# loryruta/gl-radix-sort

Hardware: AMD Instinct MI355X
Metric: Mkeys/s sorting 2^28 uint32 key+val; % HBM roofline; 1/2/4/8 GPU (higher is better)
Workload: dtype u32; 1 GPU; 2^28 uint32 key + uint32 val pairs, uniform-random full-range keys, vals=iota, in-place stable radix sort, 1x MI355X; pairs_per_gpu=268435456, key_distribution=uniform, parallelism=single, device=AMD Radeon Graphics (gfx950:sramecc+:xnack-), 256 CUs, 288.0 GiB, device 0

## Files before the change

### gl-radix-sort_amd/csrc/glu_hip.hip

```cpp
#include <hip/hip_runtime.h>

#include <algorithm>
#include <chrono>
#include <cmath>
#include <cstdarg>
#include <cstdio>
#include <cstdlib>
#include <cstring>
#include <mutex>
#include <string>
#include <strings.h>
#include <unordered_map>
#include <vector>

#include "glu_host.hpp"
#include "glu_sort_launch.hpp"
#include "glu_sort_object.hpp"
#include "radix_sort_kernels.hpp"
#include "radix_scatter_lines.hpp"
#include "radix_pair_passes.hpp"
#include "radix_seg_passes.hpp"
#include "radix_lds_plan.hpp"

using namespace glu_hip;
// ... 284 lines not shown
                else if (!(seen & 7u) && s->finish_backoff)
                    s->finish_wait = s->finish_backoff;
            }
        }
        if (s->finish_wait)
        {
            s->finish_wait--;
            finish_kpt = 0;
        }
    }
    if (finish_kpt)
    {
        s->finish_seq = s->finish_seq >= 0x0FFFFFFFu ? 1u : s->finish_seq + 1;
        s->cur_seq = s->finish_seq;
        for (uint32_t i = num_passes; i-- > 0;) passes[i + 2] = passes[i];
        finish_top_bit = !device_top && key_xf == KEY_XF_NONE && !s->no_bit_shortcut && s->finish_top ? std::min<uint32_t>(s->finish_top, end_bit) : end_bit;
        passes[0] = PassDesc{finish_top_bit - 16u, 8u, key_xf, 0};
        passes[1] = PassDesc{finish_top_bit - 8u, 8u, 0u, 0};
        num_passes += 2;
    }
    const bool finish_long_ok = finish_kpt && s->long_runs && s->long_image.ptr && finish_top_bit >= 16 &&
                                finish_top_bit - 16u <= (sizeof(KeyT) == 4 ? 16u : 48u);
    s->last_finish_long_ok = finish_long_ok;
    s->last_device_top = finish_kpt && device_top;
    s->last_finish_top = finish_kpt ? finish_top_bit : 0u;
    s->last_finish_attempted = finish_kpt != 0;
    const uint32_t finish_last = std::min<uint32_t>(finish_kpt + 2, kFinishGeometries);
    const uint32_t finish_expected = s->finish_last_geo >= finish_kpt && s->finish_last_geo <= finish_last ? s->finish_last_geo : finish_kpt;
    s->last_finish_capacity = finish_kpt ? finish_geometry_capacity(finish_last) : 0u;
    if (pairs_ok || finish_kpt)
    {
        const bool lines8 = lines_applicable<KeyT, 8>(s, kbuf[0], vbuf[0], kbuf[1], vbuf[1], count);
        const bool lines4 = lines_applicable<KeyT, 4>(s, kbuf[0], vbuf[0], kbuf[1], vbuf[1], count);
        for (uint32_t i = 0; i + 1 < num_passes;)
        {
            const bool wide = passes[i].bits > 4;
            if ((pairs_ok || (finish_kpt && i == 0)) && wide == (passes[i + 1].bits > 4) && (wide ? lines8 : lines4) &&
                ((passes[i].xform & 3u) == 0 || (finish_kpt && i == 0)))
            {
                passes[i].pair_role = 1;
                passes[i + 1].pair_role = 2;
                i += 2;
            }
            else
                i += 1;
        }
    }
    if (planned)
    {
        PassPlan* plan = (PassPlan*) s->plan.ptr;
        static_assert(offsetof(PassPlan, sample_done) + sizeof(plan->sample_done) <= sizeof(PassPlan) && offsetof(PassPlan, sample_done) + 64 > sizeof(PassPlan),
                      "sample_done is the last member of the zeroed tail of the plan");
        static_assert(offsetof(PassPlan, pair_fallback) % 64 == 0 && sizeof(PassPlan) % 64 == 0, "one aligned fill");
        HIP_TRY(hipMemsetAsync(plan->pair_fallback, 0, sizeof(PassPlan) - offsetof(PassPlan, pair_fallback), stream));
        if (finish_kpt && device_top)
        {
            hipLaunchKernelGGL((radix_sample_top_kernel<KeyT>), dim3(kSampleTopBlocks), dim3(256), 0, stream, (const KeyT*) kbuf[0], (uint32_t) count, end_bit,
                               std::min<uint32_t>(s->top_floor, end_bit), plan);
            HIP_TRY(hipGetLastError());
        }
    }
    if (planned)
        for (uint32_t i = 0; i < (uint32_t) kPlanMaxPasses; i++) s->last_pair_roles[i] = i < num_passes ? (uint32_t) passes[i].pair_role : 0u;
    const bool fork = planned && finish_kpt && s->fork_behind && !s->finish_last_refused && s->ensure_side();
    uint32_t pass = 0;
    for (; pass < num_passes; pass++)
    {
        const uint32_t shift = passes[pass].shift, bits = passes[pass].bits, xform = passes[pass].xform;
        if (planned)
        {
            PlanArgs pa;
            pa.plan = (PassPlan*) s->plan.ptr;
            pa.pass = pass;
            pa.may_skip = xform == 0;
            if (key_xf == KEY_XF_NONE && !s->no_bit_shortcut) pa.flags = pass == 0 ? kPlanCollectBits : (pa.may_skip ? kPlanShortcut : 0u);
            pa.pair_role = passes[pass].pair_role;
            if (pa.pair_role == 1)
            {
                pa.shift2 = passes[pass + 1].shift;
                pa.bits2 = passes[pass + 1].bits;
            }
            s->cur_kind = finish_kpt && pass < 2 ? 1 : 0;
            pa.behind_attempt = finish_kpt && pass >= 2;
            s->cur_behind = pa.behind_attempt;
            if (finish_kpt && pass == 0)
            {
                pa.finish_geo_first = finish_kpt;
                pa.finish_geo_last = finish_last;
                pa.finish_first_ordinary = 2;
                pa.finish_num_ordinary = num_passes - 2;
                pa.finish_seq = s->finish_seq;
                pa.finish_top_bit = finish_top_bit;
                pa.finish_key_bits = end_bit;
                pa.finish_long_ok = finish_long_ok;
                pa.fork_side = fork;
            }
            pa.unitsum_side = fork && pass == 1 && pa.pair_role == 2 && bits == 8;
            GLU_TRY(dispatch_pass<KeyT>(s, kbuf[0], vbuf[0], kbuf[1], vbuf[1], count, shift, bits, nullptr,
                                        fork && pa.behind_attempt ? s->side : stream, xform, pa));
            {
                if (finish_kpt && pass == 1)
                {
                    if (fork) HIP_TRY(hipEventRecord(s->ev_fork2, stream));
                    s->cur_kind = 2;
                    s->cur_behind = false;
                    s->mark(stream);
                    s->mark(stream);
                    const FinishMarks finish_marks{[](void* object, hipStream_t st) { ((glu_radix_sort_s*) object)->mark(st, true); }, s};
// ... 1162 lines not shown
```

### gl-radix-sort_amd/csrc/glu_sort_passes.hpp

```cpp
#pragma once
#include "glu_sort_object.hpp"
#include "radix_scatter_lines.hpp"
#include "radix_pair_passes.hpp"
#include "radix_lds_plan.hpp"

namespace glu_hip
{
namespace host
{
template<typename KeyT, int BITS, bool LARGE, bool XF, bool VALS>
glu_status launch_pass(glu_radix_sort_s* s, const KeyT* src_k, const uint32_t* src_v, KeyT* dst_k, uint32_t* dst_v,
                       size_t count, uint32_t shift, uint32_t bits, uint32_t* histogram_out, hipStream_t stream,
                       uint32_t xform = 0, PlanArgs pa = PlanArgs())
{
    using G = GeometryFor<KeyT, BITS, LARGE, VALS>;
    constexpr int RADIX = 1 << BITS;
    const uint32_t tiles = (uint32_t) ((count + G::TILE - 1) / G::TILE);
    uint64_t cap = (uint64_t) usable_cus(s) * G::BLOCKS_PER_CU;
    if (s->max_blocks) cap = std::min<uint64_t>(cap, s->max_blocks);
    const uint32_t nb = (uint32_t) std::max<uint64_t>(1, std::min<uint64_t>(tiles, cap));
    const uint32_t mask = (1u << bits) - 1;
    uint32_t* table = (uint32_t*) s->table.ptr;
    uint32_t* totals = table + (size_t) RADIX * nb;

// ... 106 lines not shown
            }
            else
            {
                auto count4_plain = radix_pair4_count_kernel<KeyT, G::TILE, false, false>;
                auto count4_collect = radix_pair4_count_kernel<KeyT, G::TILE, false, true>;
                hipLaunchKernelGGL((pa.flags & kPlanCollectBits) ? count4_collect : count4_plain,
                                   dim3(nb * kPairSub), dim3(256), 0, stream, src_k, sub_table, (uint32_t*) s->pair_t2.ptr, (uint32_t) count, shift, mask, pa.shift2,
                                   (1u << pa.bits2) - 1, tiles, xform, (const KeyT*) dst_k, pa.plan, pa.pass, pa.flags, share);
            }
            HIP_TRY(hipGetLastError());
        }
    }
    if (pa.pair_role == 2)
    {
        uint32_t* leader_table = table;
        table = (uint32_t*) s->pair_table.ptr;
        totals = table + (size_t) RADIX * nb;
        ranges = (const uint2*) s->pair_ranges.ptr;
        if constexpr (BITS == 8)
        {
            hipLaunchKernelGGL(radix_pair_unitsum_kernel, dim3(nb), dim3(1024), 0, pa.unitsum_side ? s->side : stream, (const uint32_t*) s->pair_t2.ptr,
                               (const uint32_t*) leader_table, (const uint32_t*) (leader_table + (size_t) RADIX * nb), table,
                               (uint2*) s->pair_ranges.ptr, (uint32_t) count, pa.plan, pa.pass, shift, mask, pa.flags);
            if (pa.unitsum_side)
            {
                HIP_TRY(hipEventRecord(s->ev_unit, s->side));
                HIP_TRY(hipStreamWaitEvent(stream, s->ev_unit, 0));
            }
        }
        else
            hipLaunchKernelGGL(radix_pair4_unitsum_kernel, dim3(nb), dim3(1024), 0, stream, (const uint32_t*) s->pair_t2.ptr,
                               (const uint32_t*) sub_table, (const uint32_t*) (leader_table + (size_t) RADIX * nb), table,
                               (uint2*) s->pair_ranges.ptr, (uint32_t) count, pa.plan, pa.pass, shift, mask, pa.flags);
        HIP_TRY(hipGetLastError());
    }
    if (pa.pair_role != 1)
    {
        auto count_plain = radix_count_kernel<KeyT, BITS, 1024, G::TILE, XF, false>;
        auto count_collect = radix_count_kernel<KeyT, BITS, 1024, G::TILE, XF, !XF>;
        hipLaunchKernelGGL((pa.flags & kPlanCollectBits) ? count_collect : count_plain, dim3(nb), dim3(1024), 0, stream, src_k, table,
                           (uint32_t) count, shift, mask, tiles, xform, (const KeyT*) dst_k, pa.plan, pa.pass, pa.pair_role == 2,
                           pa.flags, share);
        HIP_TRY(hipGetLastError());
    }
    s->mark(stream);
    if (BITS == 4 && pa.pair_role == 1)
    {
        hipLaunchKernelGGL((radix_row_scan_kernel<256>), dim3(RADIX), dim3(256), 0, stream, sub_table, totals, nb * kPairSub,
                           (uint32_t) count, pa.may_skip ? pa.plan : (PassPlan*) nullptr, pa.pass, 0u, pa.plan, table,
                           kPairSub);
    }
    else
    {
        hipLaunchKernelGGL((radix_row_scan_kernel<256>), dim3(RADIX), dim3(256), 0, stream, table, totals, nb, (uint32_t) count,
                           pa.may_skip ? pa.plan : (PassPlan*) nullptr, pa.pass,
                           pa.pair_role == 1 && BITS == 8
                               ? (s->pair_unit_div ? std::max<uint32_t>(1u, (uint32_t) (count / nb / s->pair_unit_div)) : 0xFFFFFFFFu)
                               : 0u,
                           pa.plan);
    }
    HIP_TRY(hipGetLastError());
    if (pa.finish_geo_first)
    {
        hipLaunchKernelGGL(radix_finish_lengths_kernel, dim3(kPairRadix), dim3(1024), 0, stream, (const uint32_t*) s->pair_t2.ptr, nb,
                           (uint32_t*) s->finish_lengths.ptr, (const PassPlan*) pa.plan, pa.pass, (const uint32_t*) s->pair_wide.ptr);
        HIP_TRY(hipGetLastError());
        const bool long_runs = pa.finish_long_ok && s->long_image.ptr;
        hipLaunchKernelGGL(radix_finish_plan_kernel, dim3(kFinishPlanBlocks), dim3(1024), 0, stream, (const uint32_t*) s->finish_lengths.ptr,
                           (uint32_t*) s->finish_starts.ptr, (uint32_t) count, pa.finish_geo_first, pa.finish_geo_last, pa.plan, pa.pass,
                           pa.finish_first_ordinary, pa.finish_num_ordinary, s->finish_hint, pa.finish_seq, pa.finish_top_bit,
                           pa.finish_key_bits, long_runs ? 1u : 0u, (uint32_t*) s->finish_crowded.ptr, (uint32_t*) s->finish_outcomes.ptr,
                           (uint32_t) (sizeof(KeyT) + (VALS ? sizeof(uint32_t) : 0)));
        HIP_TRY(hipGetLastError());
        if (long_runs)
        {
            hipLaunchKernelGGL(radix_finish_long_runs_kernel, dim3(1), dim3(1024), 0, stream, (const uint32_t*) s->finish_starts.ptr,
                               (const PassPlan*) pa.plan, usable_cus(s) * kLongRunsSharesPerWg, (uint32_t*) s->long_image.ptr, (uint32_t*) s->long_hdr.ptr);
            HIP_TRY(hipGetLastError());
        }
        if (pa.fork_side)
        {
            HIP_TRY(hipEventRecord(s->ev_fork, stream));
            HIP_TRY(hipStreamWaitEvent(s->side, s->ev_fork, 0));
        }
    }
    s->mark(stream, true);
    if (histogram_out)
    {
        HIP_TRY(hipMemcpyAsync(histogram_out, totals, ((size_t) 1 << bits) * sizeof(uint32_t), hipMemcpyDeviceToDevice,
                               stream));
        if (s->after_histogram_event) HIP_TRY(hipEventRecord(s->after_histogram_event, stream));
    }
    hipLaunchKernelGGL(scatter, dim3(nb), dim3(G::THREADS), sizeof(Smem), stream, src_k, src_v, dst_k, dst_v,
                       (const uint32_t*) table, (const uint32_t*) totals, (uint32_t) count, shift, mask, tiles,
                       (unsigned long long*) nullptr, xform, pa.plan, pa.pass, ranges, share, (const uint32_t*) nullptr, (const uint32_t*) nullptr, 0u, 0u, (const uint32_t*) nullptr);
    s->mark(stream, true);
    HIP_TRY(hipGetLastError());
    return GLU_OK;
}

template<typename KeyT, int BITS>
glu_status launch_pass_sized(glu_radix_sort_s* s, const KeyT* src_k, const uint32_t* src_v, KeyT* dst_k, uint32_t* dst_v,
                             size_t count, uint32_t shift, uint32_t bits, uint32_t* histogram_out, hipStream_t stream,
                             uint32_t xform = 0, PlanArgs pa = PlanArgs())
{
    const bool vals = src_v != nullptr;
    const size_t large_tile = vals ? GeometryFor<KeyT, BITS, true, true>::TILE : GeometryFor<KeyT, BITS, true, false>::TILE;
    const bool large = count >= large_tiles_from<KeyT, BITS>(s, vals, large_tile) && !s->force_small;
    {
        if (lines_applicable<KeyT, BITS>(s, src_k, src_v, dst_k, dst_v, count))
        {
#define GLU_LAUNCH_LINES(XF_, VALS_) \
    launch_pass_lines<KeyT, BITS, XF_, VALS_>(s, src_k, src_v, dst_k, dst_v, count, shift, bits, histogram_out, stream, XF_ ? xform : 0u, pa)
            if (vals) return xform ? GLU_LAUNCH_LINES(true, true) : GLU_LAUNCH_LINES(false, true);
            return xform ? GLU_LAUNCH_LINES(true, false) : GLU_LAUNCH_LINES(false, false);
#undef GLU_LAUNCH_LINES
        }
    }
#define GLU_LAUNCH(LARGE_, XF_, VALS_) \
// ... 22 lines not shown
```

### gl-radix-sort_amd/csrc/radix_lds_plan.hpp

```cpp
#pragma once

#include "radix_lds_finish.hpp"
#include "radix_pair_passes.hpp"

namespace glu_hip
{
constexpr uint32_t kSampleTopBlocks = 64;
template<typename KeyT>
__global__ __launch_bounds__(256) void radix_sample_top_kernel(const KeyT* __restrict__ keys, uint32_t n, uint32_t key_bits,
                                                               uint32_t floor_top, PassPlan* plan)
{
    typedef uint32_t u32x4_t __attribute__((ext_vector_type(4)));
    __shared__ uint32_t red[4][4];
    const uint32_t tid = threadIdx.x, lane = tid & 63, wave = tid >> 6;
    constexpr uint32_t W = sizeof(KeyT) / 4;
    const uint64_t nvec = (uint64_t) n * sizeof(KeyT) / 16;
    const uint32_t total = gridDim.x * 256u;
    const uint32_t samples = (uint32_t) (nvec < total ? nvec : total);
    const uint64_t stride = samples ? nvec / samples : 1;
    uint32_t o[2] = {0, 0}, no[2] = {0, 0};
    const uint32_t j = blockIdx.x * 256u + tid;
    if (j < samples)
    {
        const u32x4_t x = reinterpret_cast<const u32x4_t*>(keys)[(uint64_t) j * stride];
        if (W == 1)
        {
            o[0] = x.x | x.y | x.z | x.w;
            no[0] = ~x.x | ~x.y | ~x.z | ~x.w;
        }
        else
        {
            o[0] = x.x | x.z;
            no[0] = ~x.x | ~x.z;
            o[1] = x.y | x.w;
            no[1] = ~x.y | ~x.w;
        }
    }
    if (blockIdx.x == 0 && tid == 0 && n)
    {
        const KeyT f = keys[0], l = keys[n - 1];
        o[0] |= (uint32_t) f | (uint32_t) l;
        no[0] |= ~(uint32_t) f | ~(uint32_t) l;
        if (W == 2)
        {
            o[1] |= (uint32_t) ((uint64_t) f >> 32) | (uint32_t) ((uint64_t) l >> 32);
            no[1] |= ~(uint32_t) ((uint64_t) f >> 32) | ~(uint32_t) ((uint64_t) l >> 32);
        }
    }
#pragma unroll
    for (int s = 32; s > 0; s >>= 1)
    {
        o[0] |= __shfl_xor(o[0], s);
        o[1] |= __shfl_xor(o[1], s);
        no[0] |= __shfl_xor(no[0], s);
        no[1] |= __shfl_xor(no[1], s);
    }
    if (lane == 0) red[0][wave] = o[0], red[1][wave] = o[1], red[2][wave] = no[0], red[3][wave] = no[1];
    __syncthreads();
    if (tid == 0)
    {
        for (int w = 1; w < 4; w++) o[0] |= red[0][w], o[1] |= red[1][w], no[0] |= red[2][w], no[1] |= red[3][w];
        __hip_atomic_fetch_or(&plan->sample_or[0], o[0], __ATOMIC_RELAXED, __HIP_MEMORY_SCOPE_AGENT);
        __hip_atomic_fetch_or(&plan->sample_nor[0], no[0], __ATOMIC_RELAXED, __HIP_MEMORY_SCOPE_AGENT);
        if (W == 2)
        {
            __hip_atomic_fetch_or(&plan->sample_or[1], o[1], __ATOMIC_RELAXED, __HIP_MEMORY_SCOPE_AGENT);
            __hip_atomic_fetch_or(&plan->sample_nor[1], no[1], __ATOMIC_RELAXED, __HIP_MEMORY_SCOPE_AGENT);
        }
        const uint32_t done = __hip_atomic_fetch_add(&plan->sample_done, 1u, __ATOMIC_ACQ_REL, __HIP_MEMORY_SCOPE_AGENT);
        if (done + 1 == gridDim.x)
        {
            const uint32_t vo0 = __hip_atomic_load(&plan->sample_or[0], __ATOMIC_RELAXED, __HIP_MEMORY_SCOPE_AGENT);
            const uint32_t vn0 = __hip_atomic_load(&plan->sample_nor[0], __ATOMIC_RELAXED, __HIP_MEMORY_SCOPE_AGENT);
            const uint32_t vo1 = W == 2 ? __hip_atomic_load(&plan->sample_or[1], __ATOMIC_RELAXED, __HIP_MEMORY_SCOPE_AGENT) : 0u;
            const uint32_t vn1 = W == 2 ? __hip_atomic_load(&plan->sample_nor[1], __ATOMIC_RELAXED, __HIP_MEMORY_SCOPE_AGENT) : 0u;
            const uint64_t varying = (uint64_t) (vo0 & vn0) | ((uint64_t) (vo1 & vn1) << 32);
            uint32_t top = varying ? 64u - (uint32_t) __builtin_clzll(varying) : 0u;
            top = max(max(top, floor_top), 16u);
            top = min(top, key_bits);
            if (W == 2 && top > 32 && top < 48 && top != 40) top = top < 40 ? 40u : 48u;
            plan->top_bit = top;
            plan->shift_down[0] = plan->shift_down[1] = key_bits - top;
        }
    }
}

constexpr uint32_t kLongRunsMax = 8192;
constexpr uint32_t kLongRunsMinShare = 4096;
constexpr uint32_t kLongRunsSharesPerWg = 8;

struct LongRunsLayout
{
    uint32_t nwg, off_first, off_list, off_start, words;
    __host__ __device__ explicit LongRunsLayout(uint32_t nwg_) : nwg(nwg_)
    {
        off_first = 2u * (kLongRunsMax + nwg);
        off_list = off_first + nwg + 1u;
        off_start = off_list + kLongRunsMax + 1u;
        words = off_start + kLongRunsMax;
    }
};
__device__ __forceinline__ void finish_list_long_runs(const uint32_t* starts, uint32_t geo, uint32_t finish_longest, uint32_t nwg ,
                                                      uint32_t* __restrict__ image, uint32_t* __restrict__ hdr, uint32_t (&wsum)[2][16])
{
    const LongRunsLayout lay(nwg);
    const uint32_t tid = threadIdx.x, lane = tid & 63, wave = tid >> 6;
    const uint32_t cap = finish_geometry_capacity(geo);
    constexpr uint32_t PER = kFinishRuns / 1024;
    auto ld = [&](uint32_t i) { return starts[i]; };
    if (geo == 0 || finish_longest <= cap)
    {
        if (tid < 4) hdr[tid] = tid < 3 ? 0u : nwg;
        return;
    }
    for (uint32_t w = tid; w <= nwg; w += 1024) image[lay.off_first + w] = 0xFFFFFFFFu;
    uint32_t cnt = 0, len = 0;
    {
        uint32_t a = ld(tid * PER);
        for (uint32_t j = 0; j < PER; j++)
        {
            const uint32_t e = ld(tid * PER + j + 1);
            if (e - a > cap) cnt++, len += e - a;
            a = e;
        }
    }
    auto block_exclusive = [&](uint32_t v, int slot, uint32_t& total) -> uint32_t {
        uint32_t wtotal;
        uint32_t excl = wave_exclusive_sum(v, lane, wtotal);
// ... 26 lines not shown
    const uint32_t per_wg = (uint32_t) min<uint64_t>(kLongRunsSharesPerWg, max<uint64_t>(1ull, (uint64_t) total * 64ull / ((uint64_t) finish_longest * wgs)));
    nwg = wgs * per_wg;
    if (tid == 0) hdr[3] = nwg;
    const uint32_t share = max((total + nwg - 1) / nwg, kLongRunsMinShare);
    uint32_t subs = 0;
    {
        uint32_t a = ld(tid * PER), p = pos;
        for (uint32_t j = 0; j < PER; j++)
        {
            const uint32_t e = ld(tid * PER + j + 1), l = e - a;
            if (l > cap)
            {
                subs += (p + l - 1) / share - p / share + 1;
                p += l;
            }
            a = e;
        }
    }
    uint32_t nsb;
    uint32_t sb = block_exclusive(subs, 0, nsb);
    {
        uint32_t a = ld(tid * PER), p = pos, g = seg;
        for (uint32_t j = 0; j < PER; j++)
        {
            const uint32_t e = ld(tid * PER + j + 1), l = e - a;
            if (l > cap)
            {
                image[lay.off_list + g] = sb;
                image[lay.off_start + g] = a;
                for (uint32_t w = p / share; w <= (p + l - 1) / share; w++)
                {
                    const uint32_t b0 = max(p, w * share), b1 = min(p + l, (w + 1) * share);
                    image[2 * sb] = a + (b0 - p);
                    image[2 * sb + 1] = a + (b1 - p);
                    if (b0 == w * share) image[lay.off_first + w] = sb;
                    sb++;
                }
                p += l;
                g++;
            }
            a = e;
        }
    }
    __syncthreads();
    if (tid == 0)
    {
        hdr[1] = nsb;
        image[lay.off_list + nseg] = nsb;
    }
    for (uint32_t w = tid; w <= nwg; w += 1024)
        if (image[lay.off_first + w] == 0xFFFFFFFFu) image[lay.off_first + w] = nsb;
}

static __global__ __launch_bounds__(1024) void radix_finish_lengths_kernel(const uint32_t* __restrict__ t2, uint32_t nb,
                                                                    uint32_t* __restrict__ lengths, const PassPlan* plan,
                                                                    uint32_t pass, const uint32_t* __restrict__ wide = nullptr)
{
    if (plan->off[pass] || plan->skip[pass] == kSkipWithoutCounting) return;
    __shared__ uint32_t part[8][kPairRadix];
    __shared__ uint32_t wide_list[1024], wide_n;
    const uint32_t tid = threadIdx.x, g = tid >> 7, q = tid & 127u, d = blockIdx.x;
    uint32_t lo = 0, hi = 0;
#pragma unroll 4
    for (uint32_t b = g; b < nb; b += 8)
    {
        const uint32_t w = t2[((size_t) d * nb + b) * kPairRowWords + q];
        lo += w & 0xFFFFu;
        hi += w >> 16;
    }
    part[g][2 * q] = lo;
    part[g][2 * q + 1] = hi;
    if (tid == 0) wide_n = 0;
    __syncthreads();
    if (wide && tid < nb)
    {
        const uint32_t* hdr = wide + (size_t) tid * kPairWideStride;
        const uint32_t nw = hdr[0] <= kPairWideRows ? hdr[0] : 0u;
        for (uint32_t k = 0; k < nw; k++)
            if (hdr[1 + k] == d) wide_list[atomicAdd(&wide_n, 1u)] = (tid << 8) | k;
    }
    __syncthreads();
    if (tid < kPairRadix)
    {
        uint32_t c = 0;
#pragma unroll
        for (int k = 0; k < 8; k++) c += part[k][tid];
        for (uint32_t i = 0; i < wide_n; i++)
        {
            const uint32_t bk = wide_list[i];
            c += wide[(size_t) (bk >> 8) * kPairWideStride + 16 + (bk & 255u) * kPairRadix + tid] << 16;
        }
        lengths[tid * kPairRadix + d] = c;
    }
}

static __global__ __launch_bounds__(1024) void radix_finish_plan_kernel(const uint32_t* __restrict__ lengths, uint32_t* starts,
                                                                 uint32_t n, uint32_t geo_first, uint32_t geo_last, PassPlan* plan,
                                                                 uint32_t pass,
                                                                 uint32_t first_ordinary, uint32_t num_ordinary,
                                                                 uint32_t* hint, uint32_t attempt, uint32_t top_bit,
                                                                 uint32_t key_bits, uint32_t long_ok, uint32_t* crowded_lists,
                                                                 uint32_t* outcomes = nullptr, uint32_t pair_bytes = 8)
{
    __shared__ uint32_t tmp[3][16];
    __shared__ uint32_t over_tmp[2][kFinishGeometries][16];
    const uint32_t tid = threadIdx.x, lane = tid & 63, wave = tid >> 6, b = blockIdx.x;
    const bool tables = !(plan->off[pass] || plan->skip[pass] == kSkipWithoutCounting);
    uint32_t before = 0, all = 0, longest = 0, mine = 0;
    uint32_t over_len[kFinishGeometries] = {}, over_cnt[kFinishGeometries] = {};
    if (tables)
    {
#pragma unroll
        for (uint32_t j = 0; j < kFinishPlanBlocks; j++)
        {
            const uint32_t v = lengths[j * 1024u + tid];
            all += v;
            before += j < b ? v : 0u;
            longest = max(longest, v);
            mine = j == b ? v : mine;
            if (long_ok && b == 0)
            {
#pragma unroll
                for (uint32_t g = 0; g < kFinishGeometries; g++)
                {
                    const bool over = v > finish_geometry_capacity(g + 1);
                    over_len[g] += over ? v : 0u;
                    over_cnt[g] += over ? 1u : 0u;
                }
            }
        }
    }
    uint32_t wtotal;
    uint32_t excl = wave_exclusive_sum(mine, lane, wtotal);
#pragma unroll
    for (int o = 32; o > 0; o >>= 1)
    {
        before += __shfl_xor(before, o);
        all += __shfl_xor(all, o);
        longest = max(longest, (uint32_t) __shfl_xor(longest, o));
    }
    if (long_ok && b == 0)
    {
#pragma unroll
        for (uint32_t g = 0; g < kFinishGeometries; g++)
        {
#pragma unroll
// ... 96 lines not shown
```

### gl-radix-sort_amd/csrc/radix_pair_passes.hpp

```cpp
#pragma once

#include "radix_sort_kernels.hpp"

namespace glu_hip
{
constexpr uint32_t kPairRadix = 256;
constexpr uint32_t kPairRowWords = kPairRadix / 2;
constexpr uint32_t kPairMaxRunUnits = 2048;

__device__ __forceinline__ uint32_t pair_word(uint32_t d, uint32_t e) { return d * kPairRowWords + ((e >> 1) ^ (d & 63u)); }

struct PairCountSmem
{
    static constexpr int WAVES = 16;
    uint32_t hist1[WAVES][kPairRadix];
    uint32_t hist2[kPairRadix * kPairRowWords];
};

constexpr uint32_t kPairWideRows = 14;
constexpr uint32_t kPairWideStride = 16 + kPairWideRows * 256;

template<typename KeyT, int TILE, bool XF = false, bool COLLECT = false>
__global__ __launch_bounds__(1024) void radix_pair_count_kernel(const KeyT* __restrict__ keys_a, uint32_t* __restrict__ table,
                                                                uint32_t* __restrict__ t2, uint32_t n, uint32_t shift,
// ... 44 lines not shown
    constexpr int VEC = 16 / sizeof(KeyT);
    using VecT = typename std::conditional<sizeof(KeyT) == 4, uint4, ulonglong2>::type;
    const bool vec_ok = (reinterpret_cast<uintptr_t>(keys) & 15u) == 0;
    const uint64_t nvec = vec_ok ? (end - begin) / VEC : 0;
    const VecT* vkeys = reinterpret_cast<const VecT*>(keys + begin);
    auto count_keys = [&](auto&& add, auto collect) {
        constexpr bool kCollect = decltype(collect)::value;
        TallyRun run;
        auto tally = [&](auto peel, KeyT raw) { wave_tally_mode(peel, both_digits(raw), lane, run, add); };
        auto tally_one = [&](KeyT raw) {
            if (kCollect) acc_or |= raw, acc_and &= raw;
            add(both_digits(raw), 1u);
        };
        auto tally_vec = [&](auto peel, const VecT& a) {
            if constexpr (sizeof(KeyT) == 4)
            {
                if (kCollect) acc_or |= a.x | a.y | a.z | a.w, acc_and &= a.x & a.y & a.z & a.w;
                tally(peel, a.x); tally(peel, a.y); tally(peel, a.z); tally(peel, a.w);
            }
            else
            {
                if (kCollect) acc_or |= a.x | a.y, acc_and &= a.x & a.y;
                tally(peel, a.x); tally(peel, a.y);
            }
        };
        uint64_t vbase = 0;
        auto main_loop = [&](auto peel) {
            for (; vbase + 4 * THREADS <= nvec; vbase += 4 * THREADS)
            {
                if (wave_tally_gives_up(peel, run)) break;
                VecT a = load_streaming(&vkeys[vbase + tid]);
                VecT b = load_streaming(&vkeys[vbase + tid + THREADS]);
                VecT c = load_streaming(&vkeys[vbase + tid + 2 * THREADS]);
                VecT d = load_streaming(&vkeys[vbase + tid + 3 * THREADS]);
                tally_vec(peel, a);
                tally_vec(peel, b);
                tally_vec(peel, c);
                tally_vec(peel, d);
            }
        };
        if (4 * THREADS <= nvec) wave_tally_dispatch(both_digits(vkeys[tid].x), lane, run, main_loop, add);
        uint64_t i = begin + vbase * VEC + tid;
        for (; i + 7ull * THREADS < end; i += 8ull * THREADS)
        {
            KeyT k[8];
#pragma unroll
            for (int j = 0; j < 8; j++) k[j] = keys[i + (uint64_t) j * THREADS];
#pragma unroll
            for (int j = 0; j < 8; j++) tally_one(k[j]);
        }
        for (; i < end; i += THREADS) tally_one(keys[i]);
    };
    auto add_count = [&](uint32_t de, uint32_t c) {
        atomicAdd(&my_hist[de & 255u], c);
        atomicAdd(&s.hist2[pair_word(de & 255u, de >> 8)], c << (16u * ((de >> 8) & 1u)));
    };
    count_keys(add_count, std::integral_constant<bool, COLLECT>());
    __syncthreads();
    if (COLLECT && (plan_flags & kPlanCollectBits)) plan_publish_bits<KeyT>(plan, acc_or, acc_and, lane);

    const uint32_t nb = gridDim.x, b = blockIdx.x;
    if (tid < kPairRadix)
    {
        uint32_t c = 0;
#pragma unroll
        for (int w = 0; w < WAVES; w++) c += s.hist1[w][tid];
        table[(size_t) tid * nb + b] = c;
        s.hist1[0][tid] = c;
    }
    __syncthreads();
    bool bad = false;
    for (uint32_t d = wave; d < kPairRadix; d += WAVES)
    {
        const uint32_t j0 = lane ^ (d & 63u);
        const uint32_t w0 = s.hist2[d * kPairRowWords + lane], w1 = s.hist2[d * kPairRowWords + 64 + lane];
        uint32_t sum = (w0 & 0xFFFFu) + (w0 >> 16) + (w1 & 0xFFFFu) + (w1 >> 16);
#pragma unroll
        for (int o = 32; o > 0; o >>= 1) sum += __shfl_xor(sum, o);
        bad = bad || sum != s.hist1[0][d];
        uint32_t* row = t2 + ((size_t) d * nb + b) * kPairRowWords;
        row[j0] = w0;
        row[64 + j0] = w1;
    }
    if (bad && lane == 0 && plan) plan->pair_fallback[pass + 1] = 1;
    if (!wide) return;
    __shared__ uint32_t nwide, wide_d[kPairWideRows];
    uint32_t* const slot_of = s.hist1[1];
    uint32_t* const wide_cnt = &s.hist1[2][0];
    static_assert(2 + kPairWideRows <= PairCountSmem::WAVES, "the wide counters live in the wave-private T1 rows, which are done with");
    __syncthreads();
    for (uint32_t i = tid; i < (1u + kPairWideRows) * kPairRadix; i += THREADS) s.hist1[1][i] = 0u;
    if (tid == 0) nwide = 0;
    __syncthreads();
    for (uint32_t d = wave; d < kPairRadix; d += WAVES)
    {
        const uint32_t w0 = s.hist2[d * kPairRowWords + lane], w1 = s.hist2[d * kPairRowWords + 64 + lane];
        uint32_t sum = (w0 & 0xFFFFu) + (w0 >> 16) + (w1 & 0xFFFFu) + (w1 >> 16);
#pragma unroll
        for (int o = 32; o > 0; o >>= 1) sum += __shfl_xor(sum, o);
        if (sum != s.hist1[0][d] && lane == 0)
        {
            const uint32_t k = atomicAdd(&nwide, 1u);
            if (k < kPairWideRows) slot_of[d] = k + 1u, wide_d[k] = d;
        }
    }
    __syncthreads();
    const uint32_t nw = nwide;
    uint32_t* const hdr = wide + (size_t) b * kPairWideStride;
    bool one_value = false;
    if (COLLECT && nw != 0)
    {
        KeyT o = acc_or, a = acc_and;
#pragma unroll
        for (int sh = 32; sh > 0; sh >>= 1)
        {
            o |= (KeyT) __shfl_xor((unsigned long long) o, sh);
            a &= (KeyT) __shfl_xor((unsigned long long) a, sh);
        }
        KeyT* const wave_bits = reinterpret_cast<KeyT*>(&s.hist2[0]);
        __syncthreads();
        if (lane == 0) wave_bits[2 * wave] = o, wave_bits[2 * wave + 1] = a;
        __syncthreads();
        o = 0, a = (KeyT) ~(KeyT) 0;
        for (int w = 0; w < WAVES; w++) o |= wave_bits[2 * w], a &= wave_bits[2 * w + 1];
        one_value = o == a;
        __syncthreads();
    }
    if (nw == 0 || nw > kPairWideRows || one_value)
    {
        if (tid == 0) hdr[0] = nw == 0 ? 0u : 0xFFFFFFFFu;
        return;
    }
    auto add_wide = [&](uint32_t de, uint32_t c) {
        const uint32_t sl = slot_of[de & 255u];
        if (sl) atomicAdd(&wide_cnt[(sl - 1u) * kPairRadix + (de >> 8)], c);
    };
    count_keys(add_wide, std::false_type());
    __syncthreads();
    if (tid == 0) hdr[0] = nw;
    if (tid < nw) hdr[1 + tid] = wide_d[tid];
    for (uint32_t k = 0; k < nw; k++)
    {
        const uint32_t d = wide_d[k];
        if (tid < kPairRadix) hdr[16 + k * kPairRadix + tid] = wide_cnt[k * kPairRadix + tid] >> 16;
        if (tid < kPairRowWords)
            t2[((size_t) d * nb + b) * kPairRowWords + tid] =
                (wide_cnt[k * kPairRadix + 2 * tid] & 0xFFFFu) | (wide_cnt[k * kPairRadix + 2 * tid + 1] << 16);
    }
}


template<int RADIX>
__device__ __forceinline__ void pair_unit_bases(const uint32_t* __restrict__ totals_l, uint32_t n, uint32_t* base, uint32_t* tmp)
{
    const uint32_t tid = threadIdx.x, lane = tid & 63, wave = tid >> 6;
    const uint32_t t = tid < (uint32_t) RADIX ? totals_l[tid] : 0u;
    uint32_t wtotal;
    uint32_t excl = wave_exclusive_sum(t, lane, wtotal);
    if (lane == 0) tmp[wave] = wtotal;
    __syncthreads();
    excl += sum_of_preceding_waves(tmp, 4, wave < 4 ? wave : 0, lane);
// ... 279 lines not shown
```

### gl-radix-sort_amd/csrc/radix_sort_kernels.hpp

```cpp
#pragma once

#include <hip/hip_runtime.h>
#include <stdint.h>
#include <type_traits>

#include "device_utils.hpp"

#ifndef GLU_DMA_AUX
#define GLU_DMA_AUX 0
#endif

namespace glu_hip
{
constexpr int kWave = 64;

template<typename KeyT>
__device__ __forceinline__ uint32_t digit_of(KeyT key, uint32_t shift, uint32_t mask)
{
    const uint32_t width = (uint32_t) __popc(mask);
    if constexpr (sizeof(KeyT) == 4)
        return __builtin_amdgcn_ubfe((uint32_t) key, shift, width);
    else
    {
        const uint32_t hi_sel = shift >= 32u ? 0xFFFFFFFFu : 0u;
// ... 374 lines not shown
        {
            if (COLLECT) acc_or |= a.x | a.y, acc_and &= a.x & a.y;
            tally(peel, dig(a.x)); tally(peel, dig(a.y));
        }
    };
    uint64_t vbase = 0;
    auto main_loop = [&](auto peel) {
        for (; vbase + 4 * THREADS <= nvec; vbase += 4 * THREADS)
        {
            if (wave_tally_gives_up(peel, run)) break;
            VecT a = load_streaming(&vkeys[vbase + tid]);
            VecT b = load_streaming(&vkeys[vbase + tid + THREADS]);
            VecT c = load_streaming(&vkeys[vbase + tid + 2 * THREADS]);
            VecT d = load_streaming(&vkeys[vbase + tid + 3 * THREADS]);
            tally_vec(peel, a);
            tally_vec(peel, b);
            tally_vec(peel, c);
            tally_vec(peel, d);
        }
    };
    if (4 * THREADS <= nvec) wave_tally_dispatch(dig(vkeys[tid].x), lane, run, main_loop, add_count);
    uint64_t i = begin + vbase * VEC + tid;
    for (; i + 7ull * THREADS < end; i += 8ull * THREADS)
    {
        KeyT k[8];
#pragma unroll
        for (int j = 0; j < 8; j++) k[j] = keys[i + (uint64_t) j * THREADS];
#pragma unroll
        for (int j = 0; j < 8; j++)
        {
            if (COLLECT) acc_or |= k[j], acc_and &= k[j];
            atomicAdd(&my_hist[dig(k[j])], 1u);
        }
    }
    for (; i < end; i += THREADS)
    {
        const KeyT k = keys[i];
        if (COLLECT) acc_or |= k, acc_and &= k;
        atomicAdd(&my_hist[dig(k)], 1u);
    }
    __syncthreads();
    if (COLLECT && (plan_flags & kPlanCollectBits)) plan_publish_bits<KeyT>(plan, acc_or, acc_and, lane);

    for (int d = tid; d < RADIX; d += THREADS)
    {
        uint32_t c = 0;
#pragma unroll
        for (int w = 0; w < WAVES; w++) c += hist[w][d];
        table[(size_t) d * gridDim.x + blockIdx.x] = c;
    }
}

template<int THREADS>
__global__ __launch_bounds__(THREADS) void radix_row_scan_kernel(uint32_t* __restrict__ table,
                                                                 uint32_t* __restrict__ totals, uint32_t num_blocks,
                                                                 uint32_t n = 0, PassPlan* plan = nullptr,
                                                                 uint32_t pass = 0, uint32_t pair_limit = 0,
                                                                 PassPlan* pair_plan = nullptr,
                                                                 uint32_t* __restrict__ coarse = nullptr, uint32_t coarse_step = 1)
{
    constexpr int WAVES = THREADS / kWave;
    __shared__ uint32_t wave_sums[WAVES];
    const uint32_t tid = threadIdx.x, lane = tid & 63, wave = tid >> 6;
    const PassPlan* any_plan = plan ? plan : pair_plan;
    if (any_plan && any_plan->skip[pass] == kSkipWithoutCounting) return;
    uint32_t* row = table + (size_t) blockIdx.x * num_blocks;
    uint32_t carry = 0;
    for (uint32_t base = 0; base < num_blocks; base += THREADS)
    {
        uint32_t i = base + tid;
        uint32_t v = i < num_blocks ? row[i] : 0;
        if (pair_limit && v > pair_limit) pair_plan->pair_fallback[pass + 1] = 1;
        uint32_t wtotal;
        uint32_t excl = wave_exclusive_sum(v, lane, wtotal);
        if (lane == 0) wave_sums[wave] = wtotal;
        __syncthreads();
        uint32_t woff = 0, all = 0;
#pragma unroll
        for (int w = 0; w < WAVES; w++)
        {
            uint32_t s = wave_sums[w];
            if ((uint32_t) w < wave) woff += s;
            all += s;
        }
        if (i < num_blocks)
        {
            row[i] = carry + woff + excl;
            if (coarse && i % coarse_step == 0) coarse[(size_t) blockIdx.x * (num_blocks / coarse_step) + i / coarse_step] = carry + woff + excl;
        }
        carry += all;
        __syncthreads();
    }
    if (tid == 0)
    {
        totals[blockIdx.x] = carry;
        if (plan && carry == n) plan->skip[pass] = 1;
    }
}

template<int THREADS, int TILE, int MAX_PASSES = 4>
__global__ __launch_bounds__(THREADS) void radix_hist_kernel(const uint32_t* __restrict__ keys, uint32_t* __restrict__ ghist,
                                                             uint32_t* __restrict__ chain, uint32_t n, uint32_t passes,
                                                             uint32_t shifts, uint32_t widths)
{
    constexpr int RADIX = 256;
    __shared__ uint32_t hist[MAX_PASSES][RADIX];
    const uint32_t tid = threadIdx.x, b = blockIdx.x, tiles = gridDim.x;
    for (int i = tid; i < MAX_PASSES * RADIX; i += THREADS) (&hist[0][0])[i] = 0;
    const uint32_t row_words = (tiles + 15u) & ~15u, grow_words = (row_words / 16u + 15u) & ~15u;
    const size_t pass_words = (size_t) RADIX * (row_words + grow_words);
    for (uint32_t p = 0; p < passes; p++)
        for (uint32_t i = tid; i < (uint32_t) RADIX; i += THREADS)
        {
            chain[p * pass_words + (size_t) i * row_words + b] = 0u;
            if (b % 16u == 0u) chain[p * pass_words + (size_t) RADIX * row_words + (size_t) i * grow_words + b / 16u] = 0u;
        }
    __syncthreads();
    const uint64_t base = (uint64_t) b * TILE;
    for (uint32_t i = tid; i < (uint32_t) TILE; i += THREADS)
    {
        if (base + i < n)
        {
            const uint32_t k = keys[base + i];
            for (uint32_t p = 0; p < passes; p++)
                atomicAdd(&hist[p][__builtin_amdgcn_ubfe(k, (shifts >> (8 * p)) & 255u, (widths >> (8 * p)) & 255u)], 1u);
        }
    }
    __syncthreads();
    for (uint32_t i = tid; i < passes * RADIX; i += THREADS)
    {
        const uint32_t c = (&hist[0][0])[i];
        if (c) atomicAdd(&ghist[i], c);
    }
}

constexpr uint32_t kFusedScanMaxBlocks = 32;


template<typename KeyT, int COUNT, bool VALS = true>
struct PairArray
{
    KeyT keys[COUNT];
    __device__ __forceinline__ void put(uint32_t pos, KeyT k, uint32_t) { keys[pos] = k; }
    __device__ __forceinline__ void get(uint32_t pos, KeyT& k, uint32_t& v) const
    {
        k = keys[pos];
        v = 0u;
    }
};

// ... 697 lines not shown
```

Before: 74890 Mkeys/s.

## Fuse row scan with finish-lengths kernel, fold plan reset into sampler, defer first-digit count

Merges the per-digit row scan and the finish-lengths computation into one launch with split block roles. The plan tail is now cleared by the last workgroup of the top-bit sampler instead of a separate memset when that kernel runs. The pair count kernel now tallies only the 16-bit pair histogram at first and derives the first-digit counts from it. It re-counts the first digit only when a block's total does not match its key count, i.e. when the packed 16-bit halves overflowed. Together these remove launches and per-key atomics, at the cost of extra code paths and a rescan of the keys in the overflow case.

```diff
diff --git a/gl-radix-sort_amd/csrc/glu_hip.hip b/gl-radix-sort_amd/csrc/glu_hip.hip
--- a/gl-radix-sort_amd/csrc/glu_hip.hip
+++ b/gl-radix-sort_amd/csrc/glu_hip.hip
@@ -360,8 +360,9 @@
         static_assert(offsetof(PassPlan, sample_done) + sizeof(plan->sample_done) <= sizeof(PassPlan) && offsetof(PassPlan, sample_done) + 64 > sizeof(PassPlan),
                       "sample_done is the last member of the zeroed tail of the plan");
         static_assert(offsetof(PassPlan, pair_fallback) % 64 == 0 && sizeof(PassPlan) % 64 == 0, "one aligned fill");
-        HIP_TRY(hipMemsetAsync(plan->pair_fallback, 0, sizeof(PassPlan) - offsetof(PassPlan, pair_fallback), stream));
-        if (finish_kpt && device_top)
+        if (!(finish_kpt && device_top))
+            HIP_TRY(hipMemsetAsync(plan->pair_fallback, 0, sizeof(PassPlan) - offsetof(PassPlan, pair_fallback), stream));
+        else
         {
             hipLaunchKernelGGL((radix_sample_top_kernel<KeyT>), dim3(kSampleTopBlocks), dim3(256), 0, stream, (const KeyT*) kbuf[0], (uint32_t) count, end_bit,
                                std::min<uint32_t>(s->top_floor, end_bit), plan);
diff --git a/gl-radix-sort_amd/csrc/glu_sort_passes.hpp b/gl-radix-sort_amd/csrc/glu_sort_passes.hpp
--- a/gl-radix-sort_amd/csrc/glu_sort_passes.hpp
+++ b/gl-radix-sort_amd/csrc/glu_sort_passes.hpp
@@ -182,19 +182,20 @@
     }
     else
     {
-        hipLaunchKernelGGL((radix_row_scan_kernel<256>), dim3(RADIX), dim3(256), 0, stream, table, totals, nb, (uint32_t) count,
-                           pa.may_skip ? pa.plan : (PassPlan*) nullptr, pa.pass,
-                           pa.pair_role == 1 && BITS == 8
-                               ? (s->pair_unit_div ? std::max<uint32_t>(1u, (uint32_t) (count / nb / s->pair_unit_div)) : 0xFFFFFFFFu)
-                               : 0u,
-                           pa.plan);
+        const uint32_t pair_limit = pa.pair_role == 1 && BITS == 8
+                                        ? (s->pair_unit_div ? std::max<uint32_t>(1u, (uint32_t) (count / nb / s->pair_unit_div)) : 0xFFFFFFFFu)
+                                        : 0u;
+        if (pa.finish_geo_first)
+            hipLaunchKernelGGL(radix_row_scan_and_lengths_kernel, dim3(2 * kPairRadix), dim3(1024), 0, stream, table, totals, nb, (uint32_t) count,
+                               pa.may_skip ? pa.plan : (PassPlan*) nullptr, pa.pass, pair_limit, pa.plan, (const uint32_t*) s->pair_t2.ptr,
+                               (uint32_t*) s->finish_lengths.ptr, (const uint32_t*) s->pair_wide.ptr);
+        else
+            hipLaunchKernelGGL((radix_row_scan_kernel<256>), dim3(RADIX), dim3(256), 0, stream, table, totals, nb, (uint32_t) count,
+                               pa.may_skip ? pa.plan : (PassPlan*) nullptr, pa.pass, pair_limit, pa.plan);
     }
     HIP_TRY(hipGetLastError());
     if (pa.finish_geo_first)
     {
-        hipLaunchKernelGGL(radix_finish_lengths_kernel, dim3(kPairRadix), dim3(1024), 0, stream, (const uint32_t*) s->pair_t2.ptr, nb,
-                           (uint32_t*) s->finish_lengths.ptr, (const PassPlan*) pa.plan, pa.pass, (const uint32_t*) s->pair_wide.ptr);
-        HIP_TRY(hipGetLastError());
         const bool long_runs = pa.finish_long_ok && s->long_image.ptr;
         hipLaunchKernelGGL(radix_finish_plan_kernel, dim3(kFinishPlanBlocks), dim3(1024), 0, stream, (const uint32_t*) s->finish_lengths.ptr,
                            (uint32_t*) s->finish_starts.ptr, (uint32_t) count, pa.finish_geo_first, pa.finish_geo_last, pa.plan, pa.pass,
diff --git a/gl-radix-sort_amd/csrc/radix_lds_plan.hpp b/gl-radix-sort_amd/csrc/radix_lds_plan.hpp
--- a/gl-radix-sort_amd/csrc/radix_lds_plan.hpp
+++ b/gl-radix-sort_amd/csrc/radix_lds_plan.hpp
@@ -70,10 +70,21 @@
         const uint32_t done = __hip_atomic_fetch_add(&plan->sample_done, 1u, __ATOMIC_ACQ_REL, __HIP_MEMORY_SCOPE_AGENT);
         if (done + 1 == gridDim.x)
         {
+            constexpr uint32_t kFirst = offsetof(PassPlan, pair_fallback) / 4, kMeet = offsetof(PassPlan, sample_or) / 4;
+            static_assert(offsetof(PassPlan, sample_done) + 4 <= sizeof(PassPlan) && offsetof(PassPlan, sample_or) < offsetof(PassPlan, sample_done) &&
+                              offsetof(PassPlan, shift_down) < offsetof(PassPlan, sample_or),
+                          "the words the workgroups meet in lie behind everything else that a sort starts from zero");
             const uint32_t vo0 = __hip_atomic_load(&plan->sample_or[0], __ATOMIC_RELAXED, __HIP_MEMORY_SCOPE_AGENT);
             const uint32_t vn0 = __hip_atomic_load(&plan->sample_nor[0], __ATOMIC_RELAXED, __HIP_MEMORY_SCOPE_AGENT);
             const uint32_t vo1 = W == 2 ? __hip_atomic_load(&plan->sample_or[1], __ATOMIC_RELAXED, __HIP_MEMORY_SCOPE_AGENT) : 0u;
             const uint32_t vn1 = W == 2 ? __hip_atomic_load(&plan->sample_nor[1], __ATOMIC_RELAXED, __HIP_MEMORY_SCOPE_AGENT) : 0u;
+            uint32_t* const words = reinterpret_cast<uint32_t*>(plan);
+            for (uint32_t i = kFirst; i < kMeet; i++) words[i] = 0u;
+            __hip_atomic_store(&plan->sample_or[0], 0u, __ATOMIC_RELAXED, __HIP_MEMORY_SCOPE_AGENT);
+            __hip_atomic_store(&plan->sample_or[1], 0u, __ATOMIC_RELAXED, __HIP_MEMORY_SCOPE_AGENT);
+            __hip_atomic_store(&plan->sample_nor[0], 0u, __ATOMIC_RELAXED, __HIP_MEMORY_SCOPE_AGENT);
+            __hip_atomic_store(&plan->sample_nor[1], 0u, __ATOMIC_RELAXED, __HIP_MEMORY_SCOPE_AGENT);
+            __hip_atomic_store(&plan->sample_done, 0u, __ATOMIC_RELAXED, __HIP_MEMORY_SCOPE_AGENT);
             const uint64_t varying = (uint64_t) (vo0 & vn0) | ((uint64_t) (vo1 & vn1) << 32);
             uint32_t top = varying ? 64u - (uint32_t) __builtin_clzll(varying) : 0u;
             top = max(max(top, floor_top), 16u);
@@ -206,14 +217,14 @@
         if (image[lay.off_first + w] == 0xFFFFFFFFu) image[lay.off_first + w] = nsb;
 }
 
-static __global__ __launch_bounds__(1024) void radix_finish_lengths_kernel(const uint32_t* __restrict__ t2, uint32_t nb,
-                                                                    uint32_t* __restrict__ lengths, const PassPlan* plan,
-                                                                    uint32_t pass, const uint32_t* __restrict__ wide = nullptr)
+__device__ __forceinline__ void radix_finish_lengths_body(uint32_t d, const uint32_t* __restrict__ t2, uint32_t nb,
+                                                          uint32_t* __restrict__ lengths, const PassPlan* plan, uint32_t pass,
+                                                          const uint32_t* __restrict__ wide)
 {
     if (plan->off[pass] || plan->skip[pass] == kSkipWithoutCounting) return;
     __shared__ uint32_t part[8][kPairRadix];
     __shared__ uint32_t wide_list[1024], wide_n;
-    const uint32_t tid = threadIdx.x, g = tid >> 7, q = tid & 127u, d = blockIdx.x;
+    const uint32_t tid = threadIdx.x, g = tid >> 7, q = tid & 127u;
     uint32_t lo = 0, hi = 0;
 #pragma unroll 4
     for (uint32_t b = g; b < nb; b += 8)
@@ -246,6 +257,18 @@
         }
         lengths[tid * kPairRadix + d] = c;
     }
+}
+
+static __global__ __launch_bounds__(1024) void radix_row_scan_and_lengths_kernel(uint32_t* __restrict__ table, uint32_t* __restrict__ totals,
+                                                                          uint32_t nb, uint32_t n, PassPlan* mark_plan, uint32_t pass,
+                                                                          uint32_t pair_limit, PassPlan* plan,
+                                                                          const uint32_t* __restrict__ t2, uint32_t* __restrict__ lengths,
+                                                                          const uint32_t* __restrict__ wide)
+{
+    if (blockIdx.x < kPairRadix)
+        radix_row_scan_body<1024>(blockIdx.x, table, totals, nb, n, mark_plan, pass, pair_limit, plan, nullptr, 1u);
+    else
+        radix_finish_lengths_body(blockIdx.x - kPairRadix, t2, nb, lengths, plan, pass, wide);
 }
 
 static __global__ __launch_bounds__(1024) void radix_finish_plan_kernel(const uint32_t* __restrict__ lengths, uint32_t* starts,
diff --git a/gl-radix-sort_amd/csrc/radix_pair_passes.hpp b/gl-radix-sort_amd/csrc/radix_pair_passes.hpp
--- a/gl-radix-sort_amd/csrc/radix_pair_passes.hpp
+++ b/gl-radix-sort_amd/csrc/radix_pair_passes.hpp
@@ -120,7 +120,6 @@
         for (; i < end; i += THREADS) tally_one(keys[i]);
     };
     auto add_count = [&](uint32_t de, uint32_t c) {
-        atomicAdd(&my_hist[de & 255u], c);
         atomicAdd(&s.hist2[pair_word(de & 255u, de >> 8)], c << (16u * ((de >> 8) & 1u)));
     };
     count_keys(add_count, std::integral_constant<bool, COLLECT>());
@@ -128,6 +127,36 @@
     if (COLLECT && (plan_flags & kPlanCollectBits)) plan_publish_bits<KeyT>(plan, acc_or, acc_and, lane);
 
     const uint32_t nb = gridDim.x, b = blockIdx.x;
+    uint32_t* const block_total = &s.hist1[1][0];
+    uint32_t wave_total = 0;
+    for (uint32_t d = wave; d < kPairRadix; d += WAVES)
+    {
+        const uint32_t j0 = lane ^ (d & 63u);
+        const uint32_t w0 = s.hist2[d * kPairRowWords + lane], w1 = s.hist2[d * kPairRowWords + 64 + lane];
+        uint32_t sum = (w0 & 0xFFFFu) + (w0 >> 16) + (w1 & 0xFFFFu) + (w1 >> 16);
+#pragma unroll
+        for (int o = 32; o > 0; o >>= 1) sum += __shfl_xor(sum, o);
+        if (lane == 0) s.hist1[0][d] = sum;
+        wave_total += sum;
+        uint32_t* row = t2 + ((size_t) d * nb + b) * kPairRowWords;
+        row[j0] = w0;
+        row[64 + j0] = w1;
+    }
+    if (lane == 0) atomicAdd(block_total, wave_total);
+    __syncthreads();
+    uint32_t* const hdr = wide ? wide + (size_t) b * kPairWideStride : nullptr;
+    if (*block_total == (uint32_t) (end - begin))
+    {
+        if (tid < kPairRadix) table[(size_t) tid * nb + b] = s.hist1[0][tid];
+        if (wide && tid == 0) hdr[0] = 0u;
+        return;
+    }
+    __syncthreads();
+    for (uint32_t i = tid; i < sizeof(s.hist1) / 4; i += THREADS) (&s.hist1[0][0])[i] = 0u;
+    __syncthreads();
+    auto add_first = [&](uint32_t de, uint32_t c) { atomicAdd(&my_hist[de & 255u], c); };
+    count_keys(add_first, std::false_type());
+    __syncthreads();
     if (tid < kPairRadix)
     {
         uint32_t c = 0;
@@ -140,15 +169,11 @@
     bool bad = false;
     for (uint32_t d = wave; d < kPairRadix; d += WAVES)
     {
-        const uint32_t j0 = lane ^ (d & 63u);
         const uint32_t w0 = s.hist2[d * kPairRowWords + lane], w1 = s.hist2[d * kPairRowWords + 64 + lane];
         uint32_t sum = (w0 & 0xFFFFu) + (w0 >> 16) + (w1 & 0xFFFFu) + (w1 >> 16);
 #pragma unroll
         for (int o = 32; o > 0; o >>= 1) sum += __shfl_xor(sum, o);
         bad = bad || sum != s.hist1[0][d];
-        uint32_t* row = t2 + ((size_t) d * nb + b) * kPairRowWords;
-        row[j0] = w0;
-        row[64 + j0] = w1;
     }
     if (bad && lane == 0 && plan) plan->pair_fallback[pass + 1] = 1;
     if (!wide) return;
@@ -174,7 +199,6 @@
     }
     __syncthreads();
     const uint32_t nw = nwide;
-    uint32_t* const hdr = wide + (size_t) b * kPairWideStride;
     bool one_value = false;
     if (COLLECT && nw != 0)
     {
diff --git a/gl-radix-sort_amd/csrc/radix_sort_kernels.hpp b/gl-radix-sort_amd/csrc/radix_sort_kernels.hpp
--- a/gl-radix-sort_amd/csrc/radix_sort_kernels.hpp
+++ b/gl-radix-sort_amd/csrc/radix_sort_kernels.hpp
@@ -450,19 +450,16 @@
 }
 
 template<int THREADS>
-__global__ __launch_bounds__(THREADS) void radix_row_scan_kernel(uint32_t* __restrict__ table,
-                                                                 uint32_t* __restrict__ totals, uint32_t num_blocks,
-                                                                 uint32_t n = 0, PassPlan* plan = nullptr,
-                                                                 uint32_t pass = 0, uint32_t pair_limit = 0,
-                                                                 PassPlan* pair_plan = nullptr,
-                                                                 uint32_t* __restrict__ coarse = nullptr, uint32_t coarse_step = 1)
+__device__ __forceinline__ void radix_row_scan_body(uint32_t d, uint32_t* __restrict__ table, uint32_t* __restrict__ totals,
+                                                    uint32_t num_blocks, uint32_t n, PassPlan* plan, uint32_t pass, uint32_t pair_limit,
+                                                    PassPlan* pair_plan, uint32_t* __restrict__ coarse, uint32_t coarse_step)
 {
     constexpr int WAVES = THREADS / kWave;
     __shared__ uint32_t wave_sums[WAVES];
     const uint32_t tid = threadIdx.x, lane = tid & 63, wave = tid >> 6;
     const PassPlan* any_plan = plan ? plan : pair_plan;
     if (any_plan && any_plan->skip[pass] == kSkipWithoutCounting) return;
-    uint32_t* row = table + (size_t) blockIdx.x * num_blocks;
+    uint32_t* row = table + (size_t) d * num_blocks;
     uint32_t carry = 0;
     for (uint32_t base = 0; base < num_blocks; base += THREADS)
     {
@@ -484,16 +481,27 @@
         if (i < num_blocks)
         {
             row[i] = carry + woff + excl;
-            if (coarse && i % coarse_step == 0) coarse[(size_t) blockIdx.x * (num_blocks / coarse_step) + i / coarse_step] = carry + woff + excl;
+            if (coarse && i % coarse_step == 0) coarse[(size_t) d * (num_blocks / coarse_step) + i / coarse_step] = carry + woff + excl;
         }
         carry += all;
         __syncthreads();
     }
     if (tid == 0)
     {
-        totals[blockIdx.x] = carry;
+        totals[d] = carry;
         if (plan && carry == n) plan->skip[pass] = 1;
     }
+}
+
+template<int THREADS>
+__global__ __launch_bounds__(THREADS) void radix_row_scan_kernel(uint32_t* __restrict__ table,
+                                                                 uint32_t* __restrict__ totals, uint32_t num_blocks,
+                                                                 uint32_t n = 0, PassPlan* plan = nullptr,
+                                                                 uint32_t pass = 0, uint32_t pair_limit = 0,
+                                                                 PassPlan* pair_plan = nullptr,
+                                                                 uint32_t* __restrict__ coarse = nullptr, uint32_t coarse_step = 1)
+{
+    radix_row_scan_body<THREADS>(blockIdx.x, table, totals, num_blocks, n, plan, pass, pair_limit, pair_plan, coarse, coarse_step);
 }
 
 template<int THREADS, int TILE, int MAX_PASSES = 4>
```

Result: no change. 75330 Mkeys/s, median of 6 (+0.6%).
